# weleen/AGRL.pytorch

Hardware: AMD Instinct MI355X
Metric: frames/sec (fwd+GCN+distmat), MARS seq_len=8 (higher is better)
Workload: dtype fp16; 1 GPU; MARS seq_len=8 bs=32/GPU fp16 fwd+distmat (BASELINE configs[1]): 256x128 frames, VMGN ResNet50x2-branch + 2 graph layers, cosine distmat vs resident 12180 x 4096 gallery; global_batch=32, seq_len=8, gallery_rows_per_gpu=12180, parallelism=dp1, hip_graph=False, ranks=1, devices_visible=1, library=libagrl_hip.so, clip_batches_rotated=3, clip_bytes_rotated=301989888

## Files before the change

agrl.pytorch_amd/csrc/bottleneck_block.hip:

```cpp
#include "igemm_dev.h"

namespace {

struct BlockParams {
    const void* z;
    const void* w2;
    const float* b2;
    const void* w3;
    const float* b3;
    const void* res;
    const void* xs;
    const void* ws;
    const float* bs;
    void* out;
    const void* w1n;
    const float* b1n;
    void* zn;
    int F, H, W;
};

template <bool CAT, int CN>
__global__ __launch_bounds__(512) void bottleneck_block_kernel(const BlockParams p, int ntiles) {
    static_assert(CN == 64 || (CN == 128 && !CAT), "next conv1: 64 channels, or 128 with the identity shortcut");
    constexpr int NW = 8, PW = 10, PPIX = 100, PPIECES = 13, PATCH_BYTES = PPIECES * 1024, PJ = 2;
    constexpr int W_TAP = 64 * 128, W2_BYTES = 9 * W_TAP;
    constexpr int Y_BYTES = 64 * 128;
    constexpr int X_BYTES = CAT ? 64 * 128 : 0;
    constexpr int R_BYTES = 64 * 512;
    constexpr int NST = CN == 64 ? 5 : 6;
    constexpr int NA2 = CN / 64;
    __shared__ __attribute__((aligned(16))) unsigned char smem[W2_BYTES + 2 * PATCH_BYTES + Y_BYTES + X_BYTES + R_BYTES + 1024];
    unsigned char* s_w2 = smem;
    unsigned char* s_p = s_w2 + W2_BYTES;
    unsigned char* s_y = s_p + 2 * PATCH_BYTES;
    unsigned char* s_x = s_y + Y_BYTES;
    unsigned char* s_r = s_x + X_BYTES;
    unsigned char* s_dummy = s_r + R_BYTES;

    const int tid = threadIdx.x, lane = tid & 63;
    const int wave = __builtin_amdgcn_readfirstlane(tid >> 6);
    const int frow = lane & 15, fchunk = lane >> 4;
    const int lrow = lane >> 3, lchk = lane & 7;
    const int G = gridDim.x;
    const int tw = p.W >> 3, th = p.H >> 3;
    const unsigned char* zsrc = reinterpret_cast<const unsigned char*>(&g_zero16);
    const unsigned char* zg = reinterpret_cast<const unsigned char*>(p.z);
    const unsigned char* resg = reinterpret_cast<const unsigned char*>(p.res);
    const unsigned char* xsg = reinterpret_cast<const unsigned char*>(p.xs);

    {
        const int row = wave * 8 + lrow;
#pragma unroll
        for (int t = 0; t < 9; ++t)
            dma16(reinterpret_cast<const unsigned char*>(p.w2) + ((size_t)row * 576 + t * 64) * 2 + ((lchk ^ ((row >> 1) & 7)) << 4),
                  s_w2 + t * W_TAP + wave * 8 * 128);
    }
    const int wm2 = wave & 1, wn4 = wave >> 1;
    uint4 w3f[4][2], wsf[CAT ? 4 : 1][2], w1f[NA2][8];
#pragma unroll
    for (int a = 0; a < 4; ++a)
#pragma unroll
        for (int kk = 0; kk < 2; ++kk) {
            const size_t o = ((size_t)(wn4 * 64 + a * 16 + frow) * 64 + kk * 32 + fchunk * 8) * 2;
            w3f[a][kk] = *reinterpret_cast<const uint4*>(reinterpret_cast<const unsigned char*>(p.w3) + o);
            if constexpr (CAT) wsf[a][kk] = *reinterpret_cast<const uint4*>(reinterpret_cast<const unsigned char*>(p.ws) + o);
        }
#pragma unroll
    for (int a = 0; a < NA2; ++a)
#pragma unroll
        for (int ks = 0; ks < 8; ++ks)
            w1f[a][ks] = *reinterpret_cast<const uint4*>(reinterpret_cast<const unsigned char*>(p.w1n) +
                                                         ((size_t)(wn4 * (CN / 4) + a * 16 + frow) * 256 + ks * 32 + fchunk * 8) * 2);
    const int wm = wave & 3, wn = wave >> 2;
    float4 b2v[2], b3v[4], b1v[NA2];
#pragma unroll
    for (int a = 0; a < 2; ++a) b2v[a] = *reinterpret_cast<const float4*>(p.b2 + wn * 32 + a * 16 + fchunk * 4);
#pragma unroll
    for (int a = 0; a < 4; ++a) {
        b3v[a] = *reinterpret_cast<const float4*>(p.b3 + wn4 * 64 + a * 16 + fchunk * 4);
        if constexpr (CAT) {
            const float4 t = *reinterpret_cast<const float4*>(p.bs + wn4 * 64 + a * 16 + fchunk * 4);
            b3v[a].x += t.x; b3v[a].y += t.y; b3v[a].z += t.z; b3v[a].w += t.w;
// ... 153 lines not shown
            for (int a = 0; a < 4; ++a)
#pragma unroll
                for (int b = 0; b < 2; ++b) acc[a][b] = Frag<lp16_t>::mma(w3f[a][kk], xf[b], acc[a][b]);
        }
        if constexpr (CAT) {
#pragma unroll
            for (int kk = 0; kk < 2; ++kk) {
                uint4 xf[2];
#pragma unroll
                for (int b = 0; b < 2; ++b) xf[b] = *reinterpret_cast<const uint4*>(s_x + lds_off(wm2 * 32 + b * 16 + fr, kk * 4 + fc));
#pragma unroll
                for (int a = 0; a < 4; ++a)
#pragma unroll
                    for (int b = 0; b < 2; ++b) acc[a][b] = Frag<lp16_t>::mma(wsf[a][kk], xf[b], acc[a][b]);
            }
        } else {
            if (has_next) wait_vmcnt<PJ>();
            else wait_vmcnt<0>();
            wg_barrier();
        }
        uint2 rcell[2][4];
        if constexpr (!CAT) {
#pragma unroll
            for (int b = 0; b < 2; ++b) {
                const int px = wm2 * 32 + b * 16 + fr;
#pragma unroll
                for (int a = 0; a < 4; ++a) {
                    const int c = wn4 * 64 + a * 16 + fc * 4;
                    rcell[b][a] = *reinterpret_cast<const uint2*>(s_r + px * 512 + (((c >> 3) ^ (px & 31)) << 4) + ((c & 4) << 1));
                }
            }
        }
#pragma unroll
        for (int b = 0; b < 2; ++b) {
            const int px = wm2 * 32 + b * 16 + fr;
#pragma unroll
            for (int a = 0; a < 4; ++a) {
                const int c = wn4 * 64 + a * 16 + fc * 4;
                unsigned char* cell = s_r + px * 512 + (((c >> 3) ^ (px & 31)) << 4) + ((c & 4) << 1);
                float rr[4] = {0.f, 0.f, 0.f, 0.f};
                if constexpr (!CAT) {
                    unpack_lp16x2(rcell[b][a].x, rr[0], rr[1]);
                    unpack_lp16x2(rcell[b][a].y, rr[2], rr[3]);
                }
                float v[4];
                v[0] = relu_nan(acc[a][b][0] + b3v[a].x + rr[0]);
                v[1] = relu_nan(acc[a][b][1] + b3v[a].y + rr[1]);
                v[2] = relu_nan(acc[a][b][2] + b3v[a].z + rr[2]);
                v[3] = relu_nan(acc[a][b][3] + b3v[a].w + rr[3]);
                store4<lp16_t>(reinterpret_cast<lp16_t*>(cell), v);
            }
        }
        wg_barrier();
        {
            unsigned char* obase = reinterpret_cast<unsigned char*>(p.out) + gpix(img, oy0, ox0, 0) * 512;
#pragma unroll
            for (int i = 0; i < 4; ++i) {
                const int row = (td >> 5) + 16 * i;
                const int pch = td & 31;
                const uint4 v = *reinterpret_cast<const uint4*>(s_r + row * 512 + (pch << 4));
                if constexpr (CN == 64) *reinterpret_cast<uint4*>(obase + out_lane[i]) = v;
                else *reinterpret_cast<uint4*>(reinterpret_cast<unsigned char*>(p.out) + (gpix(img, oy0, ox0, row) * 256 + (pch ^ (row & 31)) * 8) * 2) = v;
            }
        }
        f32x4_t acc2[NA2][2];
#pragma unroll
        for (int a = 0; a < NA2; ++a)
#pragma unroll
            for (int b = 0; b < 2; ++b) acc2[a][b] = f32x4_t{0.f, 0.f, 0.f, 0.f};
        {
            uint4 x2[3][2];
            auto ld2 = [&](int ks, int slot) {
#pragma unroll
                for (int b = 0; b < 2; ++b) {
                    const int px = wm2 * 32 + b * 16 + fr;
                    x2[slot][b] = *reinterpret_cast<const uint4*>(s_r + px * 512 + (((ks * 4 + fc) ^ (px & 31)) << 4));
                }
            };
            ld2(0, 0);
            ld2(1, 1);
#pragma unroll
            for (int ks = 0; ks < 8; ++ks) {
                if (ks + 2 < 8) ld2(ks + 2, (ks + 2) % 3);
#pragma unroll
                for (int a = 0; a < NA2; ++a)
#pragma unroll
                    for (int b = 0; b < 2; ++b) acc2[a][b] = Frag<lp16_t>::mma(w1f[a][ks], x2[ks % 3][b], acc2[a][b]);
                __builtin_amdgcn_sched_barrier(0);
            }
        }
        unsigned char* sz = CN == 64 ? s_y : s_r;
        if constexpr (CN == 128) wg_barrier();
#pragma unroll
        for (int b = 0; b < 2; ++b) {
            const int px = wm2 * 32 + b * 16 + fr;
#pragma unroll
            for (int a = 0; a < NA2; ++a) {
                const int c = wn4 * (CN / 4) + a * 16 + fc * 4;
                float v[4];
                v[0] = relu_nan(acc2[a][b][0] + b1v[a].x);
                v[1] = relu_nan(acc2[a][b][1] + b1v[a].y);
                v[2] = relu_nan(acc2[a][b][2] + b1v[a].z);
                v[3] = relu_nan(acc2[a][b][3] + b1v[a].w);
                store4<lp16_t>(reinterpret_cast<lp16_t*>(sz + px * (CN * 2) + (((c >> 3) ^ (px & (CN / 8 - 1))) << 4) + ((c & 4) << 1)), v);
            }
        }
        wg_barrier();
#pragma unroll
        for (int i = 0; i < CN / 64; ++i) {
            const int row = td >> 3, pch = (td & 7) * (CN / 64) + i;
            const uint4 v = *reinterpret_cast<const uint4*>(sz + row * (CN * 2) + (pch << 4));
            *reinterpret_cast<uint4*>(reinterpret_cast<unsigned char*>(p.zn) + (gpix(img, oy0, ox0, row) * CN + (pch ^ (row & (CN / 8 - 1))) * 8) * 2) = v;
        }
    }
}

}

extern "C" int agrl_bottleneck_block(const void* z, const void* w2, const float* b2, const void* w3, const float* b3,
                                     const void* residual, const void* x_short, const void* w_short, const float* b_short,
                                     void* out, const void* w1_next, const float* b1_next, void* z_next, int F, int H, int W,
                                     int Cmid, int Cout, int Cnext, agrl_stream_t stream) {
    AGRL_CHECK_ARG(z && w2 && b2 && w3 && b3 && out && w1_next && b1_next && z_next, "agrl_bottleneck_block: null pointer");
    AGRL_CHECK_ARG((residual != nullptr) != (x_short != nullptr),
                   "agrl_bottleneck_block: pass either the residual map or the downsample conv's input, not both");
    AGRL_CHECK_ARG(!x_short || (w_short && b_short), "agrl_bottleneck_block: the downsample form needs its weights and bias");
    AGRL_CHECK_ARG(F > 0 && H > 0 && W > 0 && (H % 8) == 0 && (W % 8) == 0, "agrl_bottleneck_block: maps must be multiples of 8 x 8 (got %d x %d)", H, W);
    AGRL_CHECK_ARG(Cmid == 64 && Cout == 256 && (Cnext == 64 || (Cnext == 128 && !x_short)),
                   "agrl_bottleneck_block: built for Cmid=64, Cout=256, Cnext=64 (128 without downsample), got %d/%d/%d", Cmid, Cout, Cnext);
    AGRL_CHECK_ARG((size_t)F * H * W * 256 * 2 < (1ull << 40), "agrl_bottleneck_block: problem too large");
    const uintptr_t al = (uintptr_t)z | (uintptr_t)w2 | (uintptr_t)b2 | (uintptr_t)w3 | (uintptr_t)b3 | (uintptr_t)residual |
                         (uintptr_t)x_short | (uintptr_t)w_short | (uintptr_t)b_short | (uintptr_t)out | (uintptr_t)w1_next |
                         (uintptr_t)b1_next | (uintptr_t)z_next;
    AGRL_CHECK_ARG((al & 15) == 0, "agrl_bottleneck_block: pointers must be 16-byte aligned");
    BlockParams p;
    p.z = z; p.w2 = w2; p.b2 = b2; p.w3 = w3; p.b3 = b3; p.res = residual; p.xs = x_short; p.ws = w_short; p.bs = b_short;
    p.out = out; p.w1n = w1_next; p.b1n = b1_next; p.zn = z_next; p.F = F; p.H = H; p.W = W;
    const int ntiles = F * (H / 8) * (W / 8);
    const int grid = ntiles < 256 ? ntiles : 256;
    if (x_short) hipLaunchKernelGGL((bottleneck_block_kernel<true, 64>), dim3(grid), dim3(512), 0, (hipStream_t)stream, p, ntiles);
    else if (Cnext == 128) hipLaunchKernelGGL((bottleneck_block_kernel<false, 128>), dim3(grid), dim3(512), 0, (hipStream_t)stream, p, ntiles);
    else hipLaunchKernelGGL((bottleneck_block_kernel<false, 64>), dim3(grid), dim3(512), 0, (hipStream_t)stream, p, ntiles);
    AGRL_CHECK_LAUNCH("agrl_bottleneck_block");
    return 0;
}
```

agrl.pytorch_amd/torchreid/_hip.py:

```python
from __future__ import annotations

import ctypes as C
import os
import threading

import torch

F32 = 0
LP16 = 1
F32X3 = 2
F32H3P = 4
F32H3 = 3
FRAMES_NCHW = 0
FRAMES_NHWC = 1
METRIC_EUCLIDEAN = 0
METRIC_COSINE = 1

LP_NAME = os.environ.get("AGRL_HIP_LP16")
if LP_NAME is None:
    LP_NAME = os.environ.get("AGRL_HIP_PRECISION") if os.environ.get("AGRL_HIP_PRECISION") in ("fp16", "bf16") else "fp16"
if LP_NAME not in ("fp16", "bf16"):
    raise ValueError("AGRL_HIP_LP16 must be fp16 or bf16, not %r" % LP_NAME)
LP_DTYPE = torch.float16 if LP_NAME == "fp16" else torch.bfloat16

_HERE = os.path.dirname(os.path.abspath(__file__))
LIB_PATH = os.environ.get(
    "AGRL_HIP_LIB", os.path.normpath(os.path.join(_HERE, "..", "lib", "libagrl_hip.so" if LP_NAME == "fp16" else "libagrl_hip_bf16.so"))
)


class HipLibraryError(RuntimeError):
    """libagrl_hip.so is missing or incomplete."""


class HipKernelError(RuntimeError):
    """An entry point of libagrl_hip.so returned a non-zero status."""


_p = C.c_void_p
_i = C.c_int
_f = C.c_float

SIGNATURES = {
    "agrl_stem_conv_bn_relu_maxpool": [_p, _p, _p, _p, _i, _i, _i, _i, _p],
    "agrl_stem_conv_bn_relu_maxpool_lp16": [_p, _p, _p, _p, _i, _i, _i, _p],
    "agrl_conv2d_bn_act": [_p, _p, _p, _p, _p, _i, _i, _i, _i, _i, _i, _i, _i, _i, _i, _i, _p],
    "agrl_conv1x1_dual_split16": [_p, _p, _p, _p, _p] + [_i] * 8 + [_f, _i, _i, _p],
    "agrl_stem_split16": [_p, _p, _p, _p, _p, _i, _i, _i, _f, _p],
    "agrl_stem_conv_bn_relu_maxpool_u8": [_p, _p, _i, _p, _p, _p, _i, _i, _i, _i, _p],
    "agrl_stem_conv_bn_relu_maxpool_lp16_u8": [_p, _p, _i, _p, _p, _p, _i, _i, _i, _p],
    "agrl_stem_split16_u8": [_p, _p, _i, _p, _p, _p, _p, _i, _i, _i, _f, _p],
    "agrl_frames_normalize_u8": [_p, _p, _i, _p, _i, _i, _i, _p],
    "agrl_clip_resample_u8": [_p, _p, _p, _i, _i, _i, _i, _i, _p],
    "agrl_resample_taps_u8": [_i, _i, _p, _p, _p],
    "agrl_split16_planes": [_p, _p, C.c_longlong, _i, _i, _p],
    "agrl_split16_weight_planes": [_p, _p, C.c_longlong, _i, _f, _p],
    "agrl_split16_weights_inloop": [_p, _p, C.c_longlong, _i, _p],
    "agrl_conv1x1_split16": [_p, _p, _p, _p, _p, _i, _i, _i, _i, _f, _i, _p],
    "agrl_conv1x1_split16_dual": [_p, _p, _p, _p, _p, _i, _i, _i, _i, _i, _f, _i, _p],
    "agrl_conv1x1_split16_pool": [_p, _p, _p, _p, _p, _i, _i, _i, _i, _i, _i, C.POINTER(_i), _i, _i, _f, _i, _p],
    "agrl_conv3x3_packed_split16": [_p, _p, _p, _p, _i, _i, _i, _i, _i, _i, _f, _p],
    "agrl_conv2d_bn_act_split16": [_p, _p, _p, _p, _p] + [_i] * 10 + [_f, _i, _i, _p],
    "agrl_bottleneck_tail": [_p, _p, _p, _p, _p, _p, _p, _p, _p, _p, _p, _i, _i, _i, _i, _i, _p],
    "agrl_bottleneck_seam_packed_bytes": [_i, _i, _i],
    "agrl_bottleneck_seam_pack": [_p, _p, _p, _i, _i, _i, _p],
    "agrl_bottleneck_seam": [_p, _p, _p, _p, _p, _p, _p, _i, _i, _i, _i, _p],
    "agrl_conv3x3_packed_bytes": [_i, _i],
    "agrl_conv1x1_packed_bytes": [_i, _i],
    "agrl_conv1x1_pack": [_p, _p, _i, _i, _p],
    "agrl_conv1x1_packed_bn_act": [_p, _p, _p, _p, _p, _i, _i, _i, _i, _i, _p],
    "agrl_conv1x1_packed_res_bn_act": [_p, _p, _p, _p, _p, _i, _i, _i, _i, _p],
    "agrl_conv1x1_packed_res_pool": [_p, _p, _p, _p, _p, _p, _i, _i, _i, _i, _i, _i, C.POINTER(_i), _i, _i, _p],
    "agrl_conv1x1_packed_dual_duo": [_p, _p, _p, _p, _p, _i, _i, _i, _i, _i, _p],
    "agrl_conv1x1_packed_dual_strided": [_p, _p, _p, _p, _p, _i, _i, _i, _i, _i, _i, _i, _i, _p],
    "agrl_conv3x3_pack": [_p, _p, _i, _i, _p],
    "agrl_conv3x3_packed_bn_act": [_p, _p, _p, _p, _i, _i, _i, _i, _i, _i, _p],
    "agrl_bottleneck_block": [_p, _p, _p, _p, _p, _p, _p, _p, _p, _p, _p, _p, _p, _i, _i, _i, _i, _i, _i, _p],
    "agrl_conv1x1_dual_bn_act": [_p, _p, _p, _p, _p, _i, _i, _i, _i, _i, _p],
    "agrl_conv1x1_bn_act_pool": [_p, _p, _p, _p, _p, _p, _p, _i, _i, _i, _i, _i, _i, C.POINTER(_i), _i, _i, _p],
    "agrl_linear_nobias": [_p, _p, _p, _i, _i, _i, _i, _p],
    "agrl_part_pool": [_p, _p, _p, _p, _p, _i, _i, _i, _i, C.POINTER(_i), _i, _i, _p],
    "agrl_clip_pool": [_p, _p, _i, _i, _i, _i, _p],
    "agrl_graph_gram": [_p, _p, _i, _i, _i, _i, _p],
    "agrl_graph_pair_product": [_p, _p, _p, _p, _i, _i, _i, _p],
    "agrl_graph_finalize": [_p, _i, _p, _p, _i, _i, _i, _i, _i, _p],
    "agrl_graph_propagate": [_p, _p, _p, _p, _p, _f, _f, _f, _p, _p, _i, _i, _i, _p],
    "agrl_pam_pool": [_p, _p, _p, _p, _i, _i, _i, _i, _i, C.POINTER(_i), _i, _i, _p],
    "agrl_pam_combine": [_p, _p, _p, _f, _p, _p, _i, _i, _p],
    "agrl_pam_pool_train": [_p, _p, _p, _p, _p, _i, _i, _i, _i, _i, C.POINTER(_i), _i, _i, _p],
    "agrl_pam_pool_backward": [_p, _p, _p, _p, _p, _p, _p, _i, _i, _i, _i, _i, C.POINTER(_i), _i, _i, _p],
    "agrl_pam_combine_train": [_p, _p, _p, _p, _p, _i, _i, _p],
    "agrl_pam_combine_backward": [_p, _p, _p, _p, _p, _p, _p, _p, _i, _i, _p, C.c_size_t, _p],
    "agrl_col_sum_workspace": [_i, _i],
    "agrl_col_sum": [_p, _p, _i, _i, _p, C.c_size_t, _p],
    "agrl_graph_apply": [_p, _p, _p, _i, _i, _i, _i, _p],
    "agrl_graph_tracklet_operand": [_p, _p, _i, _p, _p, _i, _i, _i, _i, _i, _i, _i, _p],
    "agrl_graph_finalize_bits": [_p, _i, _p, _p, _i, _i, _i, _i, _i, _p],
    "agrl_pose_adjacency_bits": [_p, _p, _p, _i, _i, _i, _i, C.c_float, C.c_float, _p],
    "agrl_adjacency_pack": [_p, _p, _i, _i, _p],
    "agrl_graph_linear_mix": [_p, _p, _p, _p, _p, _f, _f, _f, _p, _i, _i, _i, _i, _p],
    "agrl_row_sqnorm": [_p, _p, _i, _i, _i, _p],
    "agrl_attn_pool_bnneck": [_p, _p, _p, _p, _p, _p, _p, _p, _p, _p, _i, _i, _i, _i, _i, _p],
    "agrl_sta_frame_stats": [_p, _p, _p, _p, _i, _i, _i, _i, _i, _p],
    "agrl_sta_fuse": [_p, _p, _p, _p, _p, _p, _i, _i, _i, _i, _i, _i, _p],
    "agrl_linear_bn_relu": [_p, _p, _p, _p, _p, _i, _i, _i, _i, _p],
    "agrl_attn_tail": [_p, _p, _p, _p, _p, _p, _p, _p, _p, _p, _p, _p, _p, _i, _i, _i, _i, _i, _p],
    "agrl_row_l2_normalize": [_p, _p, _i, _i, _i, _i, _i, _p],
    "agrl_distmat_split16": [_p, _p, _p, _p, _p, _i, _i, _i, _i, _i, _f, _p, C.c_size_t, _p],
    "agrl_distmat": [_p, _p, _p, _p, _p, _i, _i, _i, _i, _i, _i, _p, C.c_size_t, _p],
    "agrl_pose_adjacency": [_p, _p, _p, _i, _i, _i, _i, C.c_float, C.c_float, _p],
    "agrl_re_ranking_workspace": [_i, _i, _i],
    "agrl_re_ranking": [_p, _p, _p, _i, _i, _i, _i, C.c_double, _p, _i, _p, C.c_size_t, _p],
    "agrl_rank_topk": [_p, _i, _i, _i, _i, _i, _p, _p, _p],
    "agrl_distmat_topk_workspace": [_i, _i],
    "agrl_distmat_topk": [_p, _p, _p, _p, _i, _i, _i, _i, _i, _i, _i, _p, _p, _p, C.c_size_t, _p, C.c_size_t, _p],
    "agrl_rank_argsort": [_p, _i, _i, _i, _p, _p],
    "agrl_rank_mars": [_p, _p, _p, _p, _p, _i, _i, _i, _p, _p, _p],
    "agrl_rank_market1501": [_p, _i, _i, _i, _p, _p, _p, _p, _i, _p, _p, _p, _p],
    "agrl_triplet_hard_mine": [_p, _p, _i, _i, _p, _p, _p, _p, _p],
    "agrl_axpby": [_p, _p, _f, _f, _p, C.c_size_t, _p],
    "agrl_part_pool_backward": [_p, _p, _p, _p, _i, _i, _i, _i, _i, C.POINTER(_i), _i, _p],
    "agrl_attn_pool_backward": [_p, _p, _p, _i, _i, _i, _i, _p],
    "agrl_graph_matrix_backward": [_p, _i, _p, _p, _i, _i, _i, _i, _p],
    "agrl_xent_label_smooth": [_p, _p, _i, _i, _f, _p, _p, _p, _p],
    "agrl_triplet_loss": [_p, _p, _i, _i, _f, _i, _p, _p, _p, _p, _p, _p, _p, _p],
    "agrl_bn_workspace": [_i, _i],
    "agrl_bn_stats": [_p, _p, _p, _i, _i, _p, C.c_size_t, _p],
    "agrl_conv2d_stats": [_p, _p, _p, _p, C.c_size_t] + [_i] * 10 + [_p],
    "agrl_bn_stats_from_partials": [_p, _i, _i, _i, _p, _p, _p, C.c_size_t, _p],
    "agrl_bn_fold_train": [_p, _p, _p, _p, _f, _f, C.c_longlong, _p, _p, _p, _p, _p, _p, _i, _p],
# ... 124 lines not shown
```

agrl.pytorch_amd/torchreid/hip_ops.py:

```python
from __future__ import annotations

import ctypes as C
import functools
import os

import numpy as np
import torch

from . import _hip
from ._hip import F32, LP16, LP_DTYPE, LP_NAME, METRIC_COSINE, METRIC_EUCLIDEAN, call, dtype_code, ptr


import contextlib
import threading
import weakref

_MODE = threading.local()


@contextlib.contextmanager
def f32_split(on=True):
    prev = getattr(_MODE, 'split', False)
    _MODE.split = bool(on)
    try:
# ... 730 lines not shown
    if _hip.PROFILE is not None:
        _hip.PROFILE_TAG = {"flops": 2.0 * N * H * W * Cout * K,
                            "bytes": 2.0 * (x.numel() + (residual.numel() if residual is not None else 0)) + packed.numel() + 4.0 * pooled.numel()}
    with _dev(x):
        call("agrl_conv1x1_packed_res_pool", ptr(x), ptr(packed), ptr(bias), ptr(residual), ptr(pooled), ptr(pooled_lp),
             N, H, W, K, Cout, 1 if relu else 0, arr, len(splits), 1 if mean else 0, _stream(x))
    return pooled, pooled_lp


def bottleneck_tail_supported(y2, w3, w1_next, shortcut_conv=None):
    if (y2.dtype == LP_DTYPE and tuple(w3.shape) == (512, 1, 1, 128) and tuple(w1_next.shape) == (128, 1, 1, 512)
            and shortcut_conv is None):
        return True
    ok = (y2.dtype == LP_DTYPE and tuple(w3.shape) == (256, 1, 1, 64)
          and tuple(w1_next.shape) in ((64, 1, 1, 256), (128, 1, 1, 256)))
    if shortcut_conv is not None:
        ok = ok and tuple(shortcut_conv[0].shape) == (256, 1, 1, 64) and shortcut_conv[1] == 1 and w1_next.shape[0] == 64
    return ok


def bottleneck_tail(y2, w3, b3, residual, w1_next, b1_next, shortcut=None):
    N, H, W, Cmid = y2.shape
    Cout, Cnext = w3.shape[0], w1_next.shape[0]
    assert y2.dtype == LP_DTYPE and (residual is None) != (shortcut is None)
    xs = ws = bs = None
    Cshort = 0
    if shortcut is not None:
        xs, ws, bs = shortcut
        assert xs.shape[:3] == y2.shape[:3] and xs.dtype == y2.dtype
        Cshort = xs.shape[3]
    else:
        assert residual.shape == (N, H, W, Cout) and residual.dtype == y2.dtype
    out = torch.empty((N, H, W, Cout), dtype=y2.dtype, device=y2.device)
    z = torch.empty((N, H, W, Cnext), dtype=y2.dtype, device=y2.device)
    M = N * H * W
    if _hip.PROFILE is not None:
        rd = (residual.numel() if residual is not None else xs.numel() + ws.numel())
        _hip.PROFILE_TAG = {"flops": 2.0 * M * ((Cmid + Cshort) * Cout + Cout * Cnext),
                            "bytes": 2.0 * (y2.numel() + rd + out.numel() + z.numel() + w3.numel() + w1_next.numel())}
    with _dev(y2):
        call("agrl_bottleneck_tail", ptr(y2), ptr(w3), ptr(b3), ptr(residual), ptr(xs), ptr(ws), ptr(bs), ptr(out),
             ptr(w1_next), ptr(b1_next), ptr(z), M, Cmid, Cout, Cnext, Cshort, _stream(y2))
    return out, z


def bottleneck_block_supported(z, w2, stride, w3, w1_next, shortcut_conv=None):
    ok = (z.dtype == LP_DTYPE and stride == 1 and tuple(w2.shape) == (64, 3, 3, 64) and tuple(w3.shape) == (256, 1, 1, 64)
          and tuple(w1_next.shape) in ((64, 1, 1, 256), (128, 1, 1, 256)) and z.shape[1] % 8 == 0 and z.shape[2] % 8 == 0)
    if shortcut_conv is not None:
        ok = ok and tuple(shortcut_conv[0].shape) == (256, 1, 1, 64) and shortcut_conv[1] == 1 and w1_next.shape[0] == 64
    return ok


def bottleneck_block(z, w2, b2, w3, b3, residual, w1_next, b1_next, shortcut=None):
    N, H, W, Cmid = z.shape
    Cout, Cnext = w3.shape[0], w1_next.shape[0]
    assert z.dtype == LP_DTYPE and (residual is None) != (shortcut is None)
    xs = ws = bs = None
    if shortcut is not None:
        xs, ws, bs = shortcut
        assert tuple(xs.shape) == (N, H, W, 64) and xs.dtype == z.dtype
    else:
        assert tuple(residual.shape) == (N, H, W, Cout) and residual.dtype == z.dtype
    out = torch.empty((N, H, W, Cout), dtype=z.dtype, device=z.device)
    zn = torch.empty((N, H, W, Cnext), dtype=z.dtype, device=z.device)
    M = N * H * W
    if _hip.PROFILE is not None:
        rd = residual.numel() if residual is not None else xs.numel() + ws.numel()
        _hip.PROFILE_TAG = {"flops": 2.0 * M * (9 * Cmid * Cmid + (Cmid + (64 if shortcut is not None else 0)) * Cout + Cout * Cnext),
                            "bytes": 2.0 * (z.numel() + rd + out.numel() + zn.numel() + w2.numel() + w3.numel() + w1_next.numel())}
    with _dev(z):
        call("agrl_bottleneck_block", ptr(z), ptr(w2), ptr(b2), ptr(w3), ptr(b3), ptr(residual), ptr(xs), ptr(ws), ptr(bs),
             ptr(out), ptr(w1_next), ptr(b1_next), ptr(zn), N, H, W, Cmid, Cout, Cnext, _stream(z))
    return out, zn


def linear_nobias(x, w):
    M, K = x.shape
    Nout, K2 = w.shape
    assert K == K2 and x.dtype == w.dtype
    y = torch.empty((M, Nout), dtype=torch.float32, device=x.device)
    if _hip.PROFILE is not None:
        _hip.PROFILE_TAG = {"flops": 2.0 * M * K * Nout, "bytes": x.element_size() * (x.numel() + w.numel()) + 4 * y.numel()}
    with _dev(x):
        call("agrl_linear_nobias", ptr(x), ptr(w), ptr(y), M, K, Nout, _gemm_code(x.dtype), _stream(x))
    return y


def part_pool(x4_1, x4_2, splits, want_lp):
    F_, h, w, Cc = x4_1.shape
    assert x4_2.shape == x4_1.shape and x4_1.dtype == x4_2.dtype
    P = int(sum(splits))
    gsum = torch.empty((F_, Cc), dtype=torch.float32, device=x4_1.device)
    nodes = torch.empty((F_, P, Cc), dtype=torch.float32, device=x4_1.device)
    nodes_lp = torch.empty((F_, P, Cc), dtype=LP_DTYPE, device=x4_1.device) if want_lp else None
    arr = (C.c_int * len(splits))(*[int(s) for s in splits])
    with _dev(x4_1):
        call("agrl_part_pool", ptr(x4_1), ptr(x4_2), ptr(gsum), ptr(nodes), ptr(nodes_lp), F_, h, w, Cc, arr,
             len(splits), dtype_code(x4_1.dtype), _stream(x4_1))
    return gsum, nodes, nodes_lp


GRAM_CSLICE = 128


def graph_matrix(f, adj, use_pose, learn_graph, mask_diag=False):
    B, V, Cc = f.shape
    G = torch.empty((B, V, V), dtype=torch.float32, device=f.device)
    gram = None
    nz = 0
    with _dev(f):
        if learn_graph:
            nz = Cc // GRAM_CSLICE
            gram = torch.empty((B, nz, V, V), dtype=torch.float32, device=f.device)
            call("agrl_graph_gram", ptr(f), ptr(gram), B, V, Cc, GRAM_CSLICE, _stream(f))
        if use_pose and adjacency_is_packed(adj):
            assert tuple(adj.shape) == (B, V, (V + 31) // 32)
            call("agrl_graph_finalize_bits", ptr(gram), nz, ptr(adj.contiguous()), ptr(G), B, V, 1, 1 if learn_graph else 0,
                 1 if mask_diag else 0, _stream(f))
            return G
        if use_pose:
            assert adj is not None and tuple(adj.shape) == (B, V, V) and adj.dtype == torch.float32
            adj = adj.contiguous()
        call("agrl_graph_finalize", ptr(gram), nz, ptr(adj) if use_pose else None, ptr(G), B, V,
             1 if use_pose else 0, 1 if learn_graph else 0, 1 if mask_diag else 0, _stream(f))
# ... 845 lines not shown
```

agrl.pytorch_amd/torchreid/models/_vmgn_hip.py:

```python
from __future__ import annotations

import os

import torch

from torchreid import hip_ops as ops
from torchreid import _hip

_PRECISIONS = {'fp32': torch.float32, ops.LP_NAME: ops.LP_DTYPE, 'bf16x3': torch.float32, 'fp16x3': torch.float32}


def _fold_conv_bn(conv, bn, dtype, split16=False):
    w = conv.weight.detach().float()
    scale = bn.weight.detach().float() / torch.sqrt(bn.running_var.detach().float() + bn.eps)
    shift = bn.bias.detach().float() - bn.running_mean.detach().float() * scale
    w = (w * scale.view(-1, 1, 1, 1)).permute(0, 2, 3, 1).contiguous()
    if split16:
        assert dtype == torch.float32
        return ops.split16_inloop_weights(w), shift.contiguous()
    return w.to(dtype).contiguous(), shift.contiguous()


def check_packed_range(pack, where="vmgn"):
    def walk(obj, path):
# ... 158 lines not shown
        Kd = wd.shape[3]
        if Kd % 128:
            return False
        t, u = ops.split16_plane_weights(torch.cat([wd.view(cout, Kd), w3.view(cout, K3c)], dim=1), segments=[Kd, K3c], pair_first=True)
        p3['dual'] = (ops.conv1x1_pack(t), u, (blk['ds'][1] + blk['c3'][1]).contiguous(), cout)
    else:
        t, u = ops.split16_plane_weights(w3.view(cout, K3c))
        p3['c3'] = (ops.conv1x1_pack(t), u, blk['c3'][1], cout)
    blk['p3'] = p3
    return True


def _run_block_planes(x3, blk, pool=None):
    p3 = blk['p3']
    xp, rop = 1, 2
    y = ops.conv1x1_split16(x3, p3['c1'][0], p3['c1'][1], p3['c1'][2], p3['c1'][3], layout=xp)
    y = ops.conv3x3_split16(y, p3['c2'][0], p3['c2'][1], p3['c2'][2], p3['c2'][3])
    if 'dual' in p3:
        assert pool is None
        d = p3['dual']
        return ops.conv1x1_split16(x3, d[0], d[1], d[2], d[3], x2=y, layout=xp | rop)
    c = p3['c3']
    if pool is not None:
        return ops.conv1x1_split16_pool(y, c[0], c[1], c[2], c[3], x3, pool[0], pool[1], layout=rop)
    return ops.conv1x1_split16(y, c[0], c[1], c[2], c[3], residual3=x3, layout=rop)


def _conv2(y, blk):
    if 'c2p' in blk and y.shape[1] % 16 == 0 and y.shape[2] % 8 == 0:
        return ops.conv3x3_packed(y, blk['c2p'], blk['c2'][1], blk['c2'][0].shape[0], True)
    return ops.conv_bn_act(y, blk['c2'][0], blk['c2'][1], blk['stride'], 1, True)


def _conv1(x, blk):
    if 'c1p' in blk and x.is_contiguous():
        return ops.conv1x1_packed_res(x, blk['c1p'], blk['c1'][1], blk['c1'][0].shape[0], None, True)
    return ops.conv_bn_act(x, blk['c1'][0], blk['c1'][1], 1, 0, True)


def _run_block_inloop(x, blk, out_planes=0):
    y = ops.conv_bn_act(x, blk['c1'][0], blk['c1'][1], 1, 0, True, out_presplit=True)
    y = ops.conv_bn_act(y, blk['c2'][0], blk['c2'][1], blk['stride'], 1, True, x_presplit=True, out_presplit=True)
    if 'dual16' in blk and x.is_contiguous():
        return ops.conv1x1_dual_split16(x, y, blk['dual16'][0], blk['dual16'][1], blk['stride'], True, x2_presplit=True, out_planes=out_planes)
    shortcut = x if blk['ds'] is None else ops.conv_bn_act(x, blk['ds'][0], blk['ds'][1], blk['ds_stride'], 0, False)
    out = ops.conv_bn_act(y, blk['c3'][0], blk['c3'][1], 1, 0, True, residual=shortcut, x_presplit=True)
    return ops.to_split16_planes(out, out_planes) if out_planes else out


def _is_inloop(blk):
    return getattr(blk['c1'][0], 'agrl_presplit', False)


def _run_trunk(a, blocks):
    z = None
    for i, blk in enumerate(blocks):
        if _is_inloop(blk):
            a = _run_block_inloop(a, blk)
            continue
        nxt = blocks[i + 1] if i + 1 < len(blocks) else None
        y = z if z is not None else ops.conv_bn_act(a, blk['c1'][0], blk['c1'][1], 1, 0, True)
        if nxt is not None:
            ds = None if blk['ds'] is None else (blk['ds'][0], blk['ds_stride'])
            if ops.bottleneck_block_supported(y, blk['c2'][0], blk['stride'], blk['c3'][0], nxt['c1'][0], ds) and (
                    ds is None or a.shape[3] == 64):
                if ds is None:
                    a, z = ops.bottleneck_block(y, blk['c2'][0], blk['c2'][1], blk['c3'][0], blk['c3'][1], a,
                                                nxt['c1'][0], nxt['c1'][1])
                else:
                    a, z = ops.bottleneck_block(y, blk['c2'][0], blk['c2'][1], blk['c3'][0], blk['c3'][1], None,
                                                nxt['c1'][0], nxt['c1'][1], shortcut=(a, blk['ds'][0], blk['ds'][1]))
                continue
        y = _conv2(y, blk)
        fusable = nxt is not None and ops.bottleneck_tail_supported(y, blk['c3'][0], nxt['c1'][0])
        if fusable and blk['ds'] is not None and ops.bottleneck_tail_supported(
                y, blk['c3'][0], nxt['c1'][0], (blk['ds'][0], blk['ds_stride'])) and a.shape[3] == 64:
            a, z = ops.bottleneck_tail(y, blk['c3'][0], blk['c3'][1], None, nxt['c1'][0], nxt['c1'][1],
                                       shortcut=(a, blk['ds'][0], blk['ds'][1]))
            continue
        if ('dualps' in blk and a.is_contiguous() and y.is_contiguous() and a.dtype == y.dtype and a.shape[0] == y.shape[0]
                and tuple(y.shape[1:3]) == tuple((d - 1) // blk['stride'] + 1 for d in a.shape[1:3])):
            a = ops.conv1x1_packed_dual_strided(a, y, blk['dualps'], blk['dualps_bias'], blk['c3'][0].shape[0], blk['stride'], True)
            z = None
            continue
        shortcut = a if blk['ds'] is None else ops.conv_bn_act(a, blk['ds'][0], blk['ds'][1], blk['ds_stride'], 0, False)
        if nxt is not None and 'seam' in blk and (y.numel() // y.shape[-1]) % 128 == 0:
            a, z = ops.bottleneck_seam(y, blk['seam'], blk['c3'][1], shortcut, nxt['c1'][1], blk['seam_dims'])
            continue
        if fusable:
            a, z = ops.bottleneck_tail(y, blk['c3'][0], blk['c3'][1], shortcut, nxt['c1'][0], nxt['c1'][1])
        else:
            a = ops.conv_bn_act(y, blk['c3'][0], blk['c3'][1], 1, 0, True, residual=shortcut)
            z = None
    return a


def _run_block(x, blk, pool=None):
    if _is_inloop(blk):
        assert pool is None
        return _run_block_inloop(x, blk)
    y = _conv1(x, blk)
    y = _conv2(y, blk)
    if (pool is None and 'dualp' in blk
            and x.shape[:3] == y.shape[:3] and x.dtype == y.dtype and x.is_contiguous() and y.is_contiguous()):
        return ops.conv1x1_packed(x, blk['dualp'], blk['dual'][1], blk['dual'][0].shape[0], True, x2=y, duo=True)
    if pool is None and 'dual' in blk and ops.conv1x1_dual_supported(x, y, blk['dual'][0]):
        return ops.conv1x1_dual(x, y, blk['dual'][0], blk['dual'][1], True)
    shortcut = x if blk['ds'] is None else ops.conv_bn_act(x, blk['ds'][0], blk['ds'][1], blk['ds_stride'], 0, False)
    duo = 'c3p' in blk and blk['ds'] is None and shortcut.is_contiguous() and y.is_contiguous()
    if pool is not None:
        if duo and tuple(y.shape[1:3]) == (16, 8):
            return ops.conv1x1_packed_res_pool(y, blk['c3p'], blk['c3'][1], blk['c3'][0].shape[0], shortcut, pool[0], pool[1], False)[0]
        return ops.conv1x1_bn_act_pool(y, blk['c3'][0], blk['c3'][1], shortcut, pool[0], pool[1], False)[0]
    if duo:
        return ops.conv1x1_packed_res(y, blk['c3p'], blk['c3'][1], blk['c3'][0].shape[0], shortcut)
    return ops.conv_bn_act(y, blk['c3'][0], blk['c3'][1], 1, 0, True, residual=shortcut)


def run_stem(frames, pack, norm=None):
    mean, std = norm if norm is not None else (ops.PIXEL_MEAN, ops.PIXEL_STD)
    if pack['stem_lp'] is not None:
        return ops.stem_lp16(frames, pack['stem_lp'], pack['stem'][1], mean, std)
    if pack.get('stem_s16') is not None:
        return ops.stem_split16(frames, pack['stem_s16'][0], pack['stem_s16'][1], pack['stem_s16'][2], pack['stem'][1], mean, std)
    return ops.stem(frames, pack['stem'][0], pack['stem'][1], pack['dtype'], mean, std)


def eval_frames(model, x):
    if x.dtype == torch.uint8:
        _, B, S, _, _ = ops.clip_frames(x)
        norm = (getattr(model, 'pixel_mean', ops.PIXEL_MEAN), getattr(model, 'pixel_std', ops.PIXEL_STD))
        return x.reshape((B * S,) + tuple(x.shape[2:])), B, S, norm
    if x.dtype != torch.float32:
        raise TypeError('frames must be float32, got {}'.format(x.dtype))
    B, S, Cc, H, W = x.shape
    return x.reshape(B * S, Cc, H, W), B, S, None

# ... 148 lines not shown
```

include/agrl_hip.h:

```cpp
#ifndef AGRL_HIP_H
#define AGRL_HIP_H

#include <stddef.h>
#include <stdint.h>

#ifdef __cplusplus
extern "C" {
#endif

#define AGRL_F32 0
#define AGRL_LP16 1
#define AGRL_BF16 AGRL_LP16
#define AGRL_F32X3 2
#define AGRL_F32H3 3
#define AGRL_F32H3P 4

#define AGRL_METRIC_EUCLIDEAN 0
#define AGRL_METRIC_COSINE 1

typedef void* agrl_stream_t;

int agrl_version(void);
const char* agrl_last_error(void);

// ... 48 lines not shown
int agrl_conv1x1_split16(const void* x, const void* packed, const float* bias, const void* residual, void* out, int M, int K3,
                         int Cout, int relu, float w_unscale, int layout, agrl_stream_t stream);
int agrl_conv1x1_split16_dual(const void* x, const void* x2, const void* packed, const float* bias, void* out, int M, int K1_3,
                              int K2_3, int Cout, int relu, float w_unscale, int layout, agrl_stream_t stream);
int agrl_conv1x1_split16_pool(const void* x, const void* packed, const float* bias, const void* residual, float* pool_out, int N,
                              int H, int W, int K3, int Cout, int relu, const int* splits, int n_splits, int mean, float w_unscale,
                              int layout, agrl_stream_t stream);
int agrl_conv3x3_packed_split16(const void* x, const void* packed, const float* bias, void* out, int N, int H, int W, int Cin3,
                                int Cout, int relu, float w_unscale, agrl_stream_t stream);

int agrl_conv1x1_dual_bn_act(const void* x1, const void* x2, const void* w, const float* bias, void* out, int M,
                             int K1, int K2, int Cout, int relu, agrl_stream_t stream);

int agrl_conv1x1_bn_act_pool(const void* x, const void* w, const float* bias, const void* residual,
                             void* out, float* pool_out, void* pool_out_lp, int N, int H, int W,
                             int Cin, int Cout, int relu, const int* splits, int n_splits, int mean,
                             agrl_stream_t stream);

int agrl_bottleneck_tail(const void* y2, const void* w3, const float* b3, const void* residual,
                         const void* x_short, const void* w_short, const float* b_short, void* out,
                         const void* w1_next, const float* b1_next, void* z, int M, int Cmid, int Cout,
                         int Cnext, int Cshort, agrl_stream_t stream);

long long agrl_bottleneck_seam_packed_bytes(int Cmid, int Cout, int Cnext);
int agrl_bottleneck_seam_pack(const void* w3, const void* w1_next, void* packed, int Cmid, int Cout, int Cnext,
                              agrl_stream_t stream);
int agrl_bottleneck_seam(const void* y2, const void* packed, const float* b3, const void* residual, void* out,
                         const float* b1_next, void* z, int M, int Cmid, int Cout, int Cnext, agrl_stream_t stream);

long long agrl_conv3x3_packed_bytes(int Cin, int Cout);
int agrl_conv3x3_pack(const void* w_ohwi, void* packed, int Cin, int Cout, agrl_stream_t stream);
int agrl_conv3x3_packed_bn_act(const void* x, const void* packed, const float* bias, void* out, int N, int H, int W, int Cin,
                               int Cout, int relu, agrl_stream_t stream);

long long agrl_conv1x1_packed_bytes(int K, int Cout);
int agrl_conv1x1_pack(const void* w, void* packed, int K, int Cout, agrl_stream_t stream);
int agrl_conv1x1_packed_bn_act(const void* x, const void* x2, const void* packed, const float* bias, void* out, int M, int K1,
                               int K2, int Cout, int relu, agrl_stream_t stream);

int agrl_conv1x1_packed_res_bn_act(const void* x, const void* packed, const float* bias, const void* residual, void* out, int M,
                                   int K, int Cout, int relu, agrl_stream_t stream);
int agrl_conv1x1_packed_res_pool(const void* x, const void* packed, const float* bias, const void* residual, float* pool_out,
                                 void* pool_out_lp, int N, int H, int W, int K, int Cout, int relu, const int* splits,
                                 int n_splits, int mean, agrl_stream_t stream);
int agrl_conv1x1_packed_dual_duo(const void* x, const void* x2, const void* packed, const float* bias, void* out, int M, int K1,
                                 int K2, int Cout, int relu, agrl_stream_t stream);
int agrl_conv1x1_packed_dual_strided(const void* x, const void* x2, const void* packed, const float* bias, void* out, int N, int Hi,
                                     int Wi, int stride, int K1, int K2, int Cout, int relu, agrl_stream_t stream);

int agrl_bottleneck_block(const void* z, const void* w2, const float* b2, const void* w3, const float* b3,
                          const void* residual, const void* x_short, const void* w_short, const float* b_short,
                          void* out, const void* w1_next, const float* b1_next, void* z_next, int F, int H, int W,
                          int Cmid, int Cout, int Cnext, agrl_stream_t stream);

int agrl_linear_nobias(const void* x, const void* w, float* y, int M, int K, int Nout,
                       int in_dtype, agrl_stream_t stream);


int agrl_pose_adjacency(const float* poses, const unsigned char* detected, float* adj, int B, int S,
                        int num_split, int pyramid_part, float height, float threshold, agrl_stream_t stream);
int agrl_pose_adjacency_bits(const float* poses, const unsigned char* detected, uint32_t* adj_bits, int B, int S, int num_split,
                             int pyramid_part, float height, float threshold, agrl_stream_t stream);
int agrl_adjacency_pack(const float* adj, uint32_t* adj_bits, int B, int V, agrl_stream_t stream);


int agrl_part_pool(const void* x4_1, const void* x4_2, float* gsum, float* nodes, void* nodes_lp,
                   int F, int h, int w, int C, const int* splits, int n_splits, int dtype,
                   agrl_stream_t stream);


int agrl_graph_gram(const float* f, float* gram_part, int B, int V, int C, int cslice,
                    agrl_stream_t stream);

int agrl_graph_finalize(const float* gram_part, int nz, const float* adj, float* G, int B, int V,
                        int use_pose, int learn_graph, int mask_diag, agrl_stream_t stream);
int agrl_graph_finalize_bits(const float* gram_part, int nz, const uint32_t* adj_bits, float* G, int B, int V, int use_pose,
                             int learn_graph, int mask_diag, agrl_stream_t stream);

int agrl_graph_apply(const float* G, const float* f, void* out, int out_dtype, int B, int V, int C, agrl_stream_t stream);
int agrl_graph_tracklet_operand(const float* f, const void* adj, int adj_packed, float* G_out, void* out, int out_dtype, int B,
                                int V, int C, int use_pose, int learn_graph, int mask_diag, agrl_stream_t stream);
int agrl_graph_linear_mix(const void* p_op, const void* w, const float* f, const float* bn_scale, const float* bn_shift,
                          float keep, float gamma, float slope, float* out, int M, int K, int Nout, int in_dtype,
                          agrl_stream_t stream);

int agrl_graph_propagate(const float* f, const float* h, const float* G, const float* bn_scale,
                         const float* bn_shift, float keep, float gamma, float slope, float* out, void* out_lp,
                         int B, int V, int C, agrl_stream_t stream);


int agrl_pam_pool(const void* x, const void* qk, float* xbar, float* xmean, int F, int h, int w, int C, int Cq,
                  const int* splits, int n_splits, int dtype, agrl_stream_t stream);

int agrl_pam_combine(const float* y, const float* bv, const float* xmean, float gamma, float* nodes, void* nodes_lp,
                     int rows, int C, agrl_stream_t stream);


int agrl_pam_pool_train(const float* x, const float* qk, float* xbar, float* xmean, float* abar, int F, int h, int w, int C,
                        int Cq, const int* splits, int n_splits, int dtype, agrl_stream_t stream);

int agrl_pam_pool_backward(const float* x, const float* qk, const float* dxbar, const float* dxmean, float* dx, float* dqk,
                           float* abar, int F, int h, int w, int C, int Cq, const int* splits, int n_splits, int dtype,
                           agrl_stream_t stream);

int agrl_pam_combine_train(const float* y, const float* bv, const float* xmean, const float* gamma, float* nodes, int rows, int C,
                           agrl_stream_t stream);
// ... 150 lines not shown
```

Before: 73570 frames/s.

## Write only stride-2 subsampled output from last layer1 bottleneck block

Adds an exit variant of the fused bottleneck block kernel. In this form the block writes only the even-pixel (stride-2) subsample of its 256-channel output, because the following block's strided shortcut/dual GEMM reads only those pixels. The trunk runner then calls that dual GEMM with stride reduced accordingly, which cuts the global write and the later read of the full-resolution activation. It adds template and trunk bookkeeping plus runtime guards that raise if the compact output reaches a consumer that does not expect it. The pipeline stage count NST is also lowered for this variant.

```diff
diff --git a/agrl.pytorch_amd/csrc/bottleneck_block.hip b/agrl.pytorch_amd/csrc/bottleneck_block.hip
--- a/agrl.pytorch_amd/csrc/bottleneck_block.hip
+++ b/agrl.pytorch_amd/csrc/bottleneck_block.hip
@@ -19,15 +19,16 @@
     int F, H, W;
 };
 
-template <bool CAT, int CN>
+template <bool CAT, int CN, bool EXIT = false>
 __global__ __launch_bounds__(512) void bottleneck_block_kernel(const BlockParams p, int ntiles) {
     static_assert(CN == 64 || (CN == 128 && !CAT), "next conv1: 64 channels, or 128 with the identity shortcut");
+    static_assert(!EXIT || CN == 128, "the exit form is the layer's last block: 128-channel next conv1");
     constexpr int NW = 8, PW = 10, PPIX = 100, PPIECES = 13, PATCH_BYTES = PPIECES * 1024, PJ = 2;
     constexpr int W_TAP = 64 * 128, W2_BYTES = 9 * W_TAP;
     constexpr int Y_BYTES = 64 * 128;
     constexpr int X_BYTES = CAT ? 64 * 128 : 0;
     constexpr int R_BYTES = 64 * 512;
-    constexpr int NST = CN == 64 ? 5 : 6;
+    constexpr int NST = EXIT ? 3 : CN == 64 ? 5 : 6;
     constexpr int NA2 = CN / 64;
     __shared__ __attribute__((aligned(16))) unsigned char smem[W2_BYTES + 2 * PATCH_BYTES + Y_BYTES + X_BYTES + R_BYTES + 1024];
     unsigned char* s_w2 = smem;
@@ -287,7 +288,13 @@
             }
         }
         wg_barrier();
-        {
+        if constexpr (EXIT) {
+            const int r16 = td >> 5, pch = td & 31;
+            const int row = ((r16 >> 2) << 4) + ((r16 & 3) << 1);
+            const size_t cpix = ((size_t)img * (p.H >> 1) + (oy0 >> 1) + (r16 >> 2)) * (p.W >> 1) + (ox0 >> 1) + (r16 & 3);
+            const uint4 v = *reinterpret_cast<const uint4*>(s_r + row * 512 + (pch << 4));
+            *reinterpret_cast<uint4*>(reinterpret_cast<unsigned char*>(p.out) + (cpix * 256 + (pch ^ (row & 31)) * 8) * 2) = v;
+        } else {
             unsigned char* obase = reinterpret_cast<unsigned char*>(p.out) + gpix(img, oy0, ox0, 0) * 512;
 #pragma unroll
             for (int i = 0; i < 4; ++i) {
@@ -350,32 +357,50 @@
     }
 }
 
-}
-
-extern "C" int agrl_bottleneck_block(const void* z, const void* w2, const float* b2, const void* w3, const float* b3,
-                                     const void* residual, const void* x_short, const void* w_short, const float* b_short,
-                                     void* out, const void* w1_next, const float* b1_next, void* z_next, int F, int H, int W,
-                                     int Cmid, int Cout, int Cnext, agrl_stream_t stream) {
-    AGRL_CHECK_ARG(z && w2 && b2 && w3 && b3 && out && w1_next && b1_next && z_next, "agrl_bottleneck_block: null pointer");
+int launch_block(const char* fn, bool exit_form, const void* z, const void* w2, const float* b2, const void* w3, const float* b3,
+                 const void* residual, const void* x_short, const void* w_short, const float* b_short, void* out,
+                 const void* w1_next, const float* b1_next, void* z_next, int F, int H, int W, int Cmid, int Cout, int Cnext,
+                 agrl_stream_t stream) {
+    AGRL_CHECK_ARG(z && w2 && b2 && w3 && b3 && out && w1_next && b1_next && z_next, "%s: null pointer", fn);
     AGRL_CHECK_ARG((residual != nullptr) != (x_short != nullptr),
-                   "agrl_bottleneck_block: pass either the residual map or the downsample conv's input, not both");
-    AGRL_CHECK_ARG(!x_short || (w_short && b_short), "agrl_bottleneck_block: the downsample form needs its weights and bias");
-    AGRL_CHECK_ARG(F > 0 && H > 0 && W > 0 && (H % 8) == 0 && (W % 8) == 0, "agrl_bottleneck_block: maps must be multiples of 8 x 8 (got %d x %d)", H, W);
+                   "%s: pass either the residual map or the downsample conv's input, not both", fn);
+    AGRL_CHECK_ARG(!x_short || (w_short && b_short), "%s: the downsample form needs its weights and bias", fn);
+    AGRL_CHECK_ARG(F > 0 && H > 0 && W > 0 && (H % 8) == 0 && (W % 8) == 0, "%s: maps must be multiples of 8 x 8 (got %d x %d)", fn, H, W);
     AGRL_CHECK_ARG(Cmid == 64 && Cout == 256 && (Cnext == 64 || (Cnext == 128 && !x_short)),
-                   "agrl_bottleneck_block: built for Cmid=64, Cout=256, Cnext=64 (128 without downsample), got %d/%d/%d", Cmid, Cout, Cnext);
-    AGRL_CHECK_ARG((size_t)F * H * W * 256 * 2 < (1ull << 40), "agrl_bottleneck_block: problem too large");
+                   "%s: built for Cmid=64, Cout=256, Cnext=64 (128 without downsample), got %d/%d/%d", fn, Cmid, Cout, Cnext);
+    AGRL_CHECK_ARG(!exit_form || (Cnext == 128 && !x_short), "%s: the compact output exists for Cnext=128 with the identity residual only (got Cnext=%d)", fn, Cnext);
+    AGRL_CHECK_ARG((size_t)F * H * W * 256 * 2 < (1ull << 40), "%s: problem too large", fn);
     const uintptr_t al = (uintptr_t)z | (uintptr_t)w2 | (uintptr_t)b2 | (uintptr_t)w3 | (uintptr_t)b3 | (uintptr_t)residual |
                          (uintptr_t)x_short | (uintptr_t)w_short | (uintptr_t)b_short | (uintptr_t)out | (uintptr_t)w1_next |
                          (uintptr_t)b1_next | (uintptr_t)z_next;
-    AGRL_CHECK_ARG((al & 15) == 0, "agrl_bottleneck_block: pointers must be 16-byte aligned");
+    AGRL_CHECK_ARG((al & 15) == 0, "%s: pointers must be 16-byte aligned", fn);
     BlockParams p;
     p.z = z; p.w2 = w2; p.b2 = b2; p.w3 = w3; p.b3 = b3; p.res = residual; p.xs = x_short; p.ws = w_short; p.bs = b_short;
     p.out = out; p.w1n = w1_next; p.b1n = b1_next; p.zn = z_next; p.F = F; p.H = H; p.W = W;
     const int ntiles = F * (H / 8) * (W / 8);
     const int grid = ntiles < 256 ? ntiles : 256;
-    if (x_short) hipLaunchKernelGGL((bottleneck_block_kernel<true, 64>), dim3(grid), dim3(512), 0, (hipStream_t)stream, p, ntiles);
+    if (exit_form) hipLaunchKernelGGL((bottleneck_block_kernel<false, 128, true>), dim3(grid), dim3(512), 0, (hipStream_t)stream, p, ntiles);
+    else if (x_short) hipLaunchKernelGGL((bottleneck_block_kernel<true, 64>), dim3(grid), dim3(512), 0, (hipStream_t)stream, p, ntiles);
     else if (Cnext == 128) hipLaunchKernelGGL((bottleneck_block_kernel<false, 128>), dim3(grid), dim3(512), 0, (hipStream_t)stream, p, ntiles);
     else hipLaunchKernelGGL((bottleneck_block_kernel<false, 64>), dim3(grid), dim3(512), 0, (hipStream_t)stream, p, ntiles);
-    AGRL_CHECK_LAUNCH("agrl_bottleneck_block");
+    AGRL_CHECK_LAUNCH(fn);
     return 0;
 }
+
+}
+
+extern "C" int agrl_bottleneck_block(const void* z, const void* w2, const float* b2, const void* w3, const float* b3,
+                                     const void* residual, const void* x_short, const void* w_short, const float* b_short,
+                                     void* out, const void* w1_next, const float* b1_next, void* z_next, int F, int H, int W,
+                                     int Cmid, int Cout, int Cnext, agrl_stream_t stream) {
+    return launch_block("agrl_bottleneck_block", false, z, w2, b2, w3, b3, residual, x_short, w_short, b_short, out, w1_next, b1_next,
+                        z_next, F, H, W, Cmid, Cout, Cnext, stream);
+}
+
+extern "C" int agrl_bottleneck_block_exit(const void* z, const void* w2, const float* b2, const void* w3, const float* b3,
+                                          const void* residual, const void* x_short, const void* w_short, const float* b_short,
+                                          void* out, const void* w1_next, const float* b1_next, void* z_next, int F, int H, int W,
+                                          int Cmid, int Cout, int Cnext, agrl_stream_t stream) {
+    return launch_block("agrl_bottleneck_block_exit", true, z, w2, b2, w3, b3, residual, x_short, w_short, b_short, out, w1_next,
+                        b1_next, z_next, F, H, W, Cmid, Cout, Cnext, stream);
+}
diff --git a/agrl.pytorch_amd/torchreid/_hip.py b/agrl.pytorch_amd/torchreid/_hip.py
--- a/agrl.pytorch_amd/torchreid/_hip.py
+++ b/agrl.pytorch_amd/torchreid/_hip.py
@@ -76,6 +76,7 @@
     "agrl_conv3x3_pack": [_p, _p, _i, _i, _p],
     "agrl_conv3x3_packed_bn_act": [_p, _p, _p, _p, _i, _i, _i, _i, _i, _i, _p],
     "agrl_bottleneck_block": [_p, _p, _p, _p, _p, _p, _p, _p, _p, _p, _p, _p, _p, _i, _i, _i, _i, _i, _i, _p],
+    "agrl_bottleneck_block_exit": [_p, _p, _p, _p, _p, _p, _p, _p, _p, _p, _p, _p, _p, _i, _i, _i, _i, _i, _i, _p],
     "agrl_conv1x1_dual_bn_act": [_p, _p, _p, _p, _p, _i, _i, _i, _i, _i, _p],
     "agrl_conv1x1_bn_act_pool": [_p, _p, _p, _p, _p, _p, _p, _i, _i, _i, _i, _i, _i, C.POINTER(_i), _i, _i, _p],
     "agrl_linear_nobias": [_p, _p, _p, _i, _i, _i, _i, _p],
diff --git a/agrl.pytorch_amd/torchreid/hip_ops.py b/agrl.pytorch_amd/torchreid/hip_ops.py
--- a/agrl.pytorch_amd/torchreid/hip_ops.py
+++ b/agrl.pytorch_amd/torchreid/hip_ops.py
@@ -806,17 +806,22 @@
     return ok
 
 
-def bottleneck_block(z, w2, b2, w3, b3, residual, w1_next, b1_next, shortcut=None):
+def bottleneck_block_exit_supported(z, w2, stride, w3, w1_next):
+    return bottleneck_block_supported(z, w2, stride, w3, w1_next) and w1_next.shape[0] == 128
+
+
+def bottleneck_block(z, w2, b2, w3, b3, residual, w1_next, b1_next, shortcut=None, exit_stride=1):
     N, H, W, Cmid = z.shape
     Cout, Cnext = w3.shape[0], w1_next.shape[0]
     assert z.dtype == LP_DTYPE and (residual is None) != (shortcut is None)
+    assert exit_stride in (1, 2) and (exit_stride == 1 or (shortcut is None and Cnext == 128 and H % 8 == 0 and W % 8 == 0))
     xs = ws = bs = None
     if shortcut is not None:
         xs, ws, bs = shortcut
         assert tuple(xs.shape) == (N, H, W, 64) and xs.dtype == z.dtype
     else:
         assert tuple(residual.shape) == (N, H, W, Cout) and residual.dtype == z.dtype
-    out = torch.empty((N, H, W, Cout), dtype=z.dtype, device=z.device)
+    out = torch.empty((N, H // exit_stride, W // exit_stride, Cout), dtype=z.dtype, device=z.device)
     zn = torch.empty((N, H, W, Cnext), dtype=z.dtype, device=z.device)
     M = N * H * W
     if _hip.PROFILE is not None:
@@ -824,7 +829,7 @@
         _hip.PROFILE_TAG = {"flops": 2.0 * M * (9 * Cmid * Cmid + (Cmid + (64 if shortcut is not None else 0)) * Cout + Cout * Cnext),
                             "bytes": 2.0 * (z.numel() + rd + out.numel() + zn.numel() + w2.numel() + w3.numel() + w1_next.numel())}
     with _dev(z):
-        call("agrl_bottleneck_block", ptr(z), ptr(w2), ptr(b2), ptr(w3), ptr(b3), ptr(residual), ptr(xs), ptr(ws), ptr(bs),
+        call("agrl_bottleneck_block_exit" if exit_stride == 2 else "agrl_bottleneck_block", ptr(z), ptr(w2), ptr(b2), ptr(w3), ptr(b3), ptr(residual), ptr(xs), ptr(ws), ptr(bs),
              ptr(out), ptr(w1_next), ptr(b1_next), ptr(zn), N, H, W, Cmid, Cout, Cnext, _stream(z))
     return out, zn
 
diff --git a/agrl.pytorch_amd/torchreid/models/_vmgn_hip.py b/agrl.pytorch_amd/torchreid/models/_vmgn_hip.py
--- a/agrl.pytorch_amd/torchreid/models/_vmgn_hip.py
+++ b/agrl.pytorch_amd/torchreid/models/_vmgn_hip.py
@@ -234,9 +234,22 @@
     return getattr(blk['c1'][0], 'agrl_presplit', False)
 
 
+def trunk_exit_stride(blocks, i, y):
+    if ops.switch('AGRL_HIP_TRUNK_EXITS') == '0' or i + 1 >= len(blocks):
+        return 1
+    blk, nxt = blocks[i], blocks[i + 1]
+    if (y.dtype != ops.LP_DTYPE or _is_inloop(blk) or _is_inloop(nxt) or blk['ds'] is not None or 'dualps' not in nxt
+            or nxt['stride'] != 2 or nxt.get('ds_stride') != 2):
+        return 1
+    return 2 if ops.bottleneck_block_exit_supported(y, blk['c2'][0], blk['stride'], blk['c3'][0], nxt['c1'][0]) else 1
+
+
 def _run_trunk(a, blocks):
     z = None
+    sub = 1
     for i, blk in enumerate(blocks):
+        if sub != 1 and ('dualps' not in blk or z is None):
+            raise RuntimeError("_run_trunk: a compact block output reached a block that does not consume it (block %d)" % i)
         if _is_inloop(blk):
             a = _run_block_inloop(a, blk)
             continue
@@ -247,8 +260,9 @@
             if ops.bottleneck_block_supported(y, blk['c2'][0], blk['stride'], blk['c3'][0], nxt['c1'][0], ds) and (
                     ds is None or a.shape[3] == 64):
                 if ds is None:
+                    sub = trunk_exit_stride(blocks, i, y)
                     a, z = ops.bottleneck_block(y, blk['c2'][0], blk['c2'][1], blk['c3'][0], blk['c3'][1], a,
-                                                nxt['c1'][0], nxt['c1'][1])
+                                                nxt['c1'][0], nxt['c1'][1], exit_stride=sub)
                 else:
                     a, z = ops.bottleneck_block(y, blk['c2'][0], blk['c2'][1], blk['c3'][0], blk['c3'][1], None,
                                                 nxt['c1'][0], nxt['c1'][1], shortcut=(a, blk['ds'][0], blk['ds'][1]))
@@ -261,10 +275,13 @@
                                        shortcut=(a, blk['ds'][0], blk['ds'][1]))
             continue
         if ('dualps' in blk and a.is_contiguous() and y.is_contiguous() and a.dtype == y.dtype and a.shape[0] == y.shape[0]
-                and tuple(y.shape[1:3]) == tuple((d - 1) // blk['stride'] + 1 for d in a.shape[1:3])):
-            a = ops.conv1x1_packed_dual_strided(a, y, blk['dualps'], blk['dualps_bias'], blk['c3'][0].shape[0], blk['stride'], True)
+                and tuple(y.shape[1:3]) == tuple((d - 1) // (blk['stride'] // sub) + 1 for d in a.shape[1:3])):
+            a = ops.conv1x1_packed_dual_strided(a, y, blk['dualps'], blk['dualps_bias'], blk['c3'][0].shape[0], blk['stride'] // sub, True)
             z = None
+            sub = 1
             continue
+        if sub != 1:
+            raise RuntimeError("_run_trunk: block %d did not take the strided dual GEMM its compact input was written for" % i)
         shortcut = a if blk['ds'] is None else ops.conv_bn_act(a, blk['ds'][0], blk['ds'][1], blk['ds_stride'], 0, False)
         if nxt is not None and 'seam' in blk and (y.numel() // y.shape[-1]) % 128 == 0:
             a, z = ops.bottleneck_seam(y, blk['seam'], blk['c3'][1], shortcut, nxt['c1'][1], blk['seam_dims'])
diff --git a/include/agrl_hip.h b/include/agrl_hip.h
--- a/include/agrl_hip.h
+++ b/include/agrl_hip.h
@@ -124,6 +124,10 @@
                           const void* residual, const void* x_short, const void* w_short, const float* b_short,
                           void* out, const void* w1_next, const float* b1_next, void* z_next, int F, int H, int W,
                           int Cmid, int Cout, int Cnext, agrl_stream_t stream);
+int agrl_bottleneck_block_exit(const void* z, const void* w2, const float* b2, const void* w3, const float* b3,
+                               const void* residual, const void* x_short, const void* w_short, const float* b_short,
+                               void* out, const void* w1_next, const float* b1_next, void* z_next, int F, int H, int W,
+                               int Cmid, int Cout, int Cnext, agrl_stream_t stream);
 
 int agrl_linear_nobias(const void* x, const void* w, float* y, int M, int K, int Nout,
                        int in_dtype, agrl_stream_t stream);
```

Result: no change. 74100 frames/s, median of 6 (+0.7%).
